# facebookresearch/mbrl-lib

Measured on AMD Instinct MI355X. Metric: candidate-steps/sec (pop×particles×horizon / plan) per CEM iter; plans/sec, higher is better.
Workload: dtype f32

## Files before the change

mbrl-lib_amd/csrc/cem.hpp:

```cpp
#pragma once
#include <type_traits>

#include "common.hpp"
#include "particle_reduce.hpp"

namespace hipets {

struct CemDev {
    int n_env;
    int pop, H, A, D;
    int K;
    float alpha, one_minus_alpha;
    int return_mean, clipped, unbiased;
    const float* totals = nullptr;
    int P = 0;
    ParticleReduce reduce{};
    const int* elite_in = nullptr;
};

__device__ __forceinline__ float philox_trunc_normal(uint32_t idx_lo, uint32_t idx_hi, uint64_t seed, uint64_t stream) {
    for (uint32_t attempt = 0; attempt < 64; ++attempt) {
        const Philox4 r = philox4x32_10(idx_lo, idx_hi, attempt, (uint32_t)stream, (uint32_t)seed,
                                        (uint32_t)(seed >> 32) ^ (uint32_t)(stream >> 32) ^ 0x5EED5EEDu);
        float n0, n1, n2, n3;
        box_muller(r.x, r.y, n0, n1);
        if (fabsf(n0) <= 2.0f) return n0;
        if (fabsf(n1) <= 2.0f) return n1;
        box_muller(r.z, r.w, n2, n3);
        if (fabsf(n2) <= 2.0f) return n2;
        if (fabsf(n3) <= 2.0f) return n3;
    }
    return 0.0f;
}

__device__ __forceinline__ float philox_normal(uint32_t idx_lo, uint32_t idx_hi, uint64_t seed, uint64_t stream) {
    const Philox4 r = philox4x32_10(idx_lo, idx_hi, 0u, (uint32_t)stream, (uint32_t)seed,
                                    (uint32_t)(seed >> 32) ^ (uint32_t)(stream >> 32) ^ 0x5EED5EEDu);
    float n0, n1;
    box_muller(r.x, r.y, n0, n1);
    return n0;
}

__global__ void cem_sample_kernel(const CemDev p, const float* __restrict__ mu, const float* __restrict__ disp,
                                  const float* __restrict__ lower, const float* __restrict__ upper,
                                  const float* __restrict__ z_in, unsigned long long seed, unsigned long long stream,
                                  float* __restrict__ population) {
    const long long i = (long long)blockIdx.x * blockDim.x + threadIdx.x;
    if (i >= (long long)p.n_env * p.pop * p.D) return;
    const int d = (int)(i % p.D);
    const int env = (int)(i / ((long long)p.pop * p.D));
    const float m = mu[env * p.D + d], v = disp[env * p.D + d], lb = lower[d], ub = upper[d];
    float x;
    if (p.clipped) {
        const float z = z_in ? z_in[i] : philox_normal((uint32_t)i, (uint32_t)(i >> 32), seed, stream);
        x = m + v * z;
        x = x > lb ? x : lb;
        x = x < ub ? x : ub;
    } else {
        const float lbd = (m - lb) / 2.0f, ubd = (ub - m) / 2.0f;
        const float mv = fminf(lbd * lbd, ubd * ubd);
        const float cv = fminf(mv, v);
        const float z = z_in ? z_in[i] : philox_trunc_normal((uint32_t)i, (uint32_t)(i >> 32), seed, stream);
        x = z * sqrtf(cv) + m;
    }
    population[i] = x;
}

#ifndef HIPETS_REFIT_SKIP
#define HIPETS_REFIT_SKIP 0
#endif
constexpr int kRefitThreads = 1024;
constexpr int kMaxPop = 8192;
constexpr int kRefitScratchBytes = 12288;
constexpr int kSelectMaxK = 1024;
constexpr int kRankSortMax = 640;

__global__ __launch_bounds__(kRefitThreads) void cem_refit_kernel(const CemDev p, float* values, const float* population, float* mu,
                                                                 float* disp, float* best_value, float* best_solution,
                                                                 int* elite_idx_out) {
    extern __shared__ __attribute__((aligned(16))) char smem[];
    {
        const int env = blockIdx.y;
        values += (size_t)env * p.pop;
        if (p.totals && !(HIPETS_REFIT_SKIP & 1)) {
            const float* tot = p.totals + (size_t)env * p.pop * p.P;
            for (int i = threadIdx.x; i < p.pop; i += kRefitThreads) values[i] = particle_value(tot + (size_t)i * p.P, 1, p.P, p.reduce);
        }
        population += (size_t)env * p.pop * p.D;
        mu += (size_t)env * p.D;
        disp += (size_t)env * p.D;
        best_value += env;
        best_solution += (size_t)env * p.D;
        if (elite_idx_out) elite_idx_out += (size_t)env * p.K;
    }
    const int* const elite_in = p.elite_in ? p.elite_in + (size_t)blockIdx.y * p.K : nullptr;
    int n2 = 1;
    while (n2 < p.pop) n2 <<= 1;
    float* key = reinterpret_cast<float*>(smem);
    int* idx = reinterpret_cast<int*>(smem + (size_t)n2 * 4);
    const int tid = threadIdx.x;
    for (int i = tid; i < n2; i += kRefitThreads) {
        float v = -INFINITY;
        if (i < p.pop) {
            v = values[i];
            if (v != v) { v = -1e-10f; values[i] = v; }
        }
        key[i] = v;
        idx[i] = i < p.pop ? i : 0x7FFFFFFF;
    }
    __syncthreads();
    if (elite_in) {
        auto in_range = [&](const int e) { return e < 0 ? 0 : (e >= p.pop ? p.pop - 1 : e); };
        const float top_key = key[in_range(elite_in[0])];
        __syncthreads();
        for (int k = tid; k < p.K; k += kRefitThreads) idx[k] = in_range(elite_in[k]);
        if (tid == 0) key[0] = top_key;
        __syncthreads();
    } else if (HIPETS_REFIT_SKIP & 2) {
    } else if (p.pop <= kRankSortMax) {
        for (int i = tid; i < p.pop; i += kRefitThreads) {
            const float ki = key[i];
            int rank = 0;
#pragma unroll 8
            for (int j = 0; j < i; ++j) rank += key[j] >= ki;
#pragma unroll 8
            for (int j = i + 1; j < p.pop; ++j) rank += key[j] > ki;
            idx[i] = rank;
        }
        __syncthreads();
        int* pos = reinterpret_cast<int*>(smem + (size_t)n2 * 8);
        for (int i = tid; i < p.pop; i += kRefitThreads) pos[idx[i]] = i;
        __syncthreads();
        float top_key = key[pos[0]];
        __syncthreads();
        for (int i = tid; i < p.pop; i += kRefitThreads) idx[i] = pos[i];
        if (tid == 0) key[0] = top_key;
        __syncthreads();
    } else if (p.K <= kSelectMaxK) {
        int* hist = reinterpret_cast<int*>(smem + (size_t)n2 * 8);
        int* ctl = hist + 256;
        int* elist = ctl + 8;
        float* ekey = reinterpret_cast<float*>(elist + kSelectMaxK);
        auto okey = [](float v) {
            const unsigned u = __float_as_uint(v + 0.0f);
            return (u & 0x80000000u) ? ~u : (u | 0x80000000u);
        };
        if (tid == 0) { ctl[0] = 0; ctl[1] = 0; ctl[2] = p.K; ctl[3] = 0; }
        for (int pass = 3; pass >= 0; --pass) {
            for (int b = tid; b < 256; b += kRefitThreads) hist[b] = 0;
            __syncthreads();
            const unsigned prefix = (unsigned)ctl[0], mask = (unsigned)ctl[1];
            for (int i = tid; i < p.pop; i += kRefitThreads) {
                const unsigned u = okey(key[i]);
                if ((u & mask) == prefix) atomicAdd(&hist[(u >> (8 * pass)) & 255u], 1);
            }
            __syncthreads();
            if (tid < 64) {
                const int h0 = hist[4 * tid], h1 = hist[4 * tid + 1], h2 = hist[4 * tid + 2], h3 = hist[4 * tid + 3];
                const int mine = h0 + h1 + h2 + h3;
                int above = mine;
#pragma unroll
                for (int d = 1; d < 64; d <<= 1) {
                    const int o = __shfl_down(above, d, 64);
                    if (tid + d < 64) above += o;
                }
                const int need = ctl[2];
                const int higher = above - mine;
                if (higher < need && need <= above) {
                    int n = need - higher, b = 4 * tid + 3;
// ... 40 lines not shown
        __syncthreads();
        if (my_pos >= 0) idx[my_pos] = my_id;
        if (my_pos == 0) key[0] = my_key;
        __syncthreads();
    } else
    for (int k = 2; k <= n2; k <<= 1) {
        for (int j = k >> 1; j > 0; j >>= 1) {
            for (int i = tid; i < n2; i += kRefitThreads) {
                const int ixj = i ^ j;
                if (ixj > i) {
                    const float ka = key[i], kb = key[ixj];
                    const int ia = idx[i], ib = idx[ixj];
                    const bool a_first = (ka > kb) || (ka == kb && ia < ib);
                    const bool up = (i & k) == 0;
                    if (up ? !a_first : a_first) {
                        key[i] = kb; key[ixj] = ka;
                        idx[i] = ib; idx[ixj] = ia;
                    }
                }
            }
            __syncthreads();
        }
    }
    if (elite_idx_out && blockIdx.x == 0)
        for (int k = tid; k < p.K; k += kRefitThreads) elite_idx_out[k] = idx[k];

    const float top = key[0];
    const bool improved = blockIdx.x == 0 && top > best_value[0];
    const int top_i = idx[0];
    __syncthreads();

    double* red = reinterpret_cast<double*>(smem + (size_t)n2 * 8);
    const int nb = (int)gridDim.x, bx = (int)blockIdx.x;
    const int Dslice = (((p.D + nb - 1) / nb + 63) / 64) * 64;
    const int d_lo = bx * Dslice, d_hi = min(p.D, d_lo + Dslice);
    int parts = kRefitThreads / Dslice;
    parts = parts < 1 ? 1 : (parts > 8 ? 8 : parts);
    const int G = kRefitThreads / parts;
    const int part = tid / G, dloc = tid % G;
    const int nu = (p.K + parts - 1) / parts;
    auto sweep = [&](const int base, auto nu_tag, auto hold_tag) __attribute__((always_inline)) {
        constexpr int NU = decltype(nu_tag)::value;
        constexpr bool HOLD = decltype(hold_tag)::value;
        const int d = base + dloc;
        const bool live = d < d_hi && part < parts;
        float mu_old = 0.f, disp_old = 0.f;
        float xv[NU];
        double s = 0.0;
        if (live) {
            if (part == 0) { mu_old = mu[d]; disp_old = disp[d]; }
            for (int k0 = part; k0 < (HOLD ? part + 1 : p.K); k0 += parts * NU) {
#pragma unroll
                for (int u = 0; u < NU; ++u) xv[u] = population[(size_t)idx[min(k0 + u * parts, p.K - 1)] * p.D + d];
#pragma unroll
                for (int u = 0; u < NU; ++u)
                    if (k0 + u * parts < p.K) s += (double)xv[u];
            }
        }
// ... 8 lines not shown
        double ss = 0.0;
        if (live) {
            for (int k0 = part; k0 < (HOLD ? part + 1 : p.K); k0 += parts * NU) {
                if constexpr (!HOLD) {
#pragma unroll
                    for (int u = 0; u < NU; ++u) xv[u] = population[(size_t)idx[min(k0 + u * parts, p.K - 1)] * p.D + d];
                }
#pragma unroll
                for (int u = 0; u < NU; ++u)
                    if (k0 + u * parts < p.K) {
                        const double dv = (double)xv[u] - mean;
                        ss += dv * dv;
                    }
            }
        }
        red[tid] = ss;
        __syncthreads();
        if (live && part == 0) {
            double var = 0.0;
            for (int q = 0; q < parts; ++q) var += red[q * G + dloc];
            var /= (double)(p.unbiased ? (p.K - 1) : p.K);
            const float new_mu = (float)mean;
            const float new_disp = p.clipped ? (float)sqrt(var) : (float)var;
            mu[d] = p.alpha * mu_old + p.one_minus_alpha * new_mu;
            disp[d] = p.alpha * disp_old + p.one_minus_alpha * new_disp;
        }
        __syncthreads();
    };
    constexpr int kBestHold = 4;
    float best_row[kBestHold];
    const bool best_held = p.D <= kBestHold * kRefitThreads;
    if (improved && best_held) {
#pragma unroll
        for (int u = 0; u < kBestHold; ++u) best_row[u] = population[(size_t)top_i * p.D + min(tid + u * kRefitThreads, p.D - 1)];
    }
    for (int base = d_lo; base < ((HIPETS_REFIT_SKIP & 4) ? d_lo : d_hi); base += G) {
        using T = std::true_type;
        using F = std::false_type;
        if (nu <= 2) sweep(base, std::integral_constant<int, 2>{}, T{});
        else if (nu <= 4) sweep(base, std::integral_constant<int, 4>{}, T{});
        else if (nu <= 8) sweep(base, std::integral_constant<int, 8>{}, T{});
        else if (nu <= 16) sweep(base, std::integral_constant<int, 16>{}, T{});
        else sweep(base, std::integral_constant<int, 16>{}, F{});
    }
    if (improved) {
        if (best_held) {
#pragma unroll
            for (int u = 0; u < kBestHold; ++u)
                if (tid + u * kRefitThreads < p.D) best_solution[tid + u * kRefitThreads] = best_row[u];
        } else {
            for (int d = tid; d < p.D; d += kRefitThreads) best_solution[d] = population[(size_t)top_i * p.D + d];
        }
        if (tid == 0) best_value[0] = top;
    }
}

inline int refit_blocks(const int D) { return D <= 128 ? 1 : (D + 127) / 128 > 8 ? 8 : (D + 127) / 128; }

__global__ void cem_init_kernel(const CemDev p, const float* x0, const float* lower, const float* upper, float* mu,
                                float* disp, float* best_value) {
    const int i = blockIdx.x * blockDim.x + threadIdx.x;
    if (i < p.n_env * p.D) {
        const int d = i % p.D;
        mu[i] = x0[i];
        const float w = upper[d] - lower[d];
        disp[i] = p.clipped ? 1.0f : (w * w) / 16.0f;
    }
    if (i < p.n_env) best_value[i] = -INFINITY;
}

}
```

mbrl-lib_amd/csrc/engine.hip:

```cpp
#include <cstdarg>
#include <cstdio>
#include <cstring>

#include "engine.hpp"

namespace hipets {

thread_local std::string g_err;
thread_local int g_err_kind = HIPETS_ERR_NONE;

int fail(const char* fmt, ...) {
    char buf[1024];
    va_list ap;
    va_start(ap, fmt);
    vsnprintf(buf, sizeof(buf), fmt, ap);
    va_end(ap);
    g_err = buf;
    g_err_kind = HIPETS_ERR_INVALID_ARGUMENT;
    return 1;
}

int fail_kind(const int kind, const char* fmt, ...) {
    char buf[1024];
    va_list ap;
// ... 69 lines not shown
    HCHECK(hipGetDeviceProperties(&prop, device));
    if (std::string(prop.gcnArchName).rfind("gfx950", 0) != 0)
        return fail("device %d is %s; libhipets is built for gfx950 (MI355X) only", device, prop.gcnArchName);
    auto* e = new hipets_engine();
    e->device = device;
    e->num_cu = prop.multiProcessorCount > 0 ? prop.multiProcessorCount : 256;
    e->lds_max = prop.sharedMemPerBlockOptin > 0 ? (size_t)prop.sharedMemPerBlockOptin : (size_t)prop.sharedMemPerBlock;
    if (e->lds_max > 160 * 1024) e->lds_max = 160 * 1024;
    if (hipHostMalloc(reinterpret_cast<void**>(&e->error_flag), sizeof(int), hipHostMallocMapped) != hipSuccess) e->error_flag = nullptr;
    if (e->error_flag) *e->error_flag = 0;
    const char* np = std::getenv("HIPETS_NO_PERSISTENT");
    e->persistent_ok = e->error_flag != nullptr && !(np && np[0] == '1');
    if (e->census.ensure(2 * sizeof(int))) e->persistent_ok = false;
    *out = e;
    return 0;
}

void hipets_destroy(hipets_engine* e) {
    if (!e) return;
    (void)hipSetDevice(e->device);
    comm_release(e);
    for (DevBuf* b : {&e->w3pack, &e->wpack, &e->bpack, &e->layer_meta, &e->norm_mean, &e->norm_std, &e->min_lv, &e->max_lv, &e->no_delta, &e->members,
                      &e->s0, &e->state, &e->totals, &e->term, &e->exchange, &e->step_keys, &e->plan_keys, &e->mu, &e->disp, &e->population, &e->values,
                      &e->best_value, &e->best_solution, &e->past_action, &e->kept, &e->elite_idx, &e->keep_idx, &e->planet_w, &e->planet_b, &e->planet_member, &e->planet_ops, &e->shard_values, &e->gathered, &e->census, &e->train_slab, &e->train_partial,
                      &e->policy.w, &e->policy.b, &e->compact_counts, &e->sac_ws, &e->sac_one, &e->critic.w, &e->critic.b,
                      &e->ensemble.w, &e->ensemble.b, &e->ensemble.norm, &e->ensemble.lv, &e->ensemble.cols})
        b->release();
    for (auto& ev : e->events) { (void)hipEventDestroy(ev.first); (void)hipEventDestroy(ev.second); }
    for (auto& ev : e->event_pool) { (void)hipEventDestroy(ev.first); (void)hipEventDestroy(ev.second); }
    if (e->error_flag) (void)hipHostFree(e->error_flag);
    if (e->last_done) (void)hipEventDestroy(e->last_done);
    for (auto& sl : e->stage) {
        if (sl.p) (void)hipHostFree(sl.p);
        if (sl.done) (void)hipEventDestroy(sl.done);
    }
    delete e;
}

int hipets_set_plan_mode(hipets_engine* e, int32_t mode) {
    if (!e) return fail("null engine");
    if (mode != HIPETS_MODE_FAST && mode != HIPETS_MODE_DEVICE) return fail("plan mode must be HIPETS_MODE_FAST or HIPETS_MODE_DEVICE");
    e->plan_mode = mode;
    return 0;
}

int hipets_set_particle_reduce(hipets_engine* e, int32_t kind, float kappa, int32_t worst_k) {
    if (!e) return fail("null engine");
// ... 74 lines not shown
```

mbrl-lib_amd/csrc/engine.hpp:

```cpp
#pragma once
#include <hip/hip_runtime.h>

#include <cstdlib>
#include <string>
#include <utility>
#include <vector>

#include "../../include/hipets.h"
#include "particle_reduce.hpp"
#include "planet_types.hpp"
#include "rollout_types.hpp"

namespace hipets {

extern thread_local std::string g_err;
extern thread_local int g_err_kind;

}

#pragma GCC visibility push(hidden)

namespace hipets {

int fail(const char* fmt, ...);
// ... 58 lines not shown
    int num_cu = 256;
    size_t lds_max = 160 * 1024;
    bool has_model = false;
    hipets::ModelDev md{};
    int ensemble_size = 0;
    DevBuf w3pack;
    DevBuf wpack, bpack, layer_meta, norm_mean, norm_std, min_lv, max_lv, no_delta, members;
    DevBuf s0, state, totals, term;
    DevBuf exchange, step_keys, plan_keys;
    struct HostStage { void* p = nullptr; size_t cap = 0; hipEvent_t done = nullptr; bool used = false; };
    HostStage stage[4];
    int stage_next = 0;
    uint32_t tag_base = 0;
    uint64_t plan_keys_seed = 0, plan_keys_first = 0;
    int plan_keys_count = 0, plan_keys_H = 0;
    int* error_flag = nullptr;
    bool persistent_ok = true;
    long long poll_ticks = 20000000ll;
    DevBuf census;
    hipStream_t last_stream = nullptr;
    bool last_stream_set = false;
    hipEvent_t last_done = nullptr;
    DevBuf mu, disp, population, values, best_value, best_solution, past_action, kept, elite_idx, keep_idx;
    void* comm = nullptr;
    int comm_rank = 0, comm_world = 1;
    DevBuf shard_values, gathered;
    bool has_planet = false;
    bool planet_static = false;
    hipets::PlanetDev pd{};
    DevBuf planet_w, planet_b, planet_member, planet_ops;
    int plan_mode = HIPETS_MODE_FAST;
    hipets::ParticleReduce reduce{};
    bool has_trace = false;
    hipets_plan_trace trace{};
    bool timing = false;
    int timing_stride = 1;
    unsigned long long launch_counter = 0;
    std::vector<std::pair<hipEvent_t, hipEvent_t>> events;
    std::vector<std::pair<hipEvent_t, hipEvent_t>> event_pool;
    DevBuf train_slab, train_partial;
    hipets::MlpSnapshot policy, critic;
    DevBuf compact_counts;
    bool has_sac = false;
    hipets::SacBind sac{};
    int sac_last_batch = 0;
    DevBuf sac_ws, sac_one;
// ... 22 lines not shown
    int kind = HIPETS_ERR_NONE;
    bool ok() const { return kind == HIPETS_ERR_NONE; }
    void note(const int rc) {
        if (rc && ok()) { msg = g_err; kind = g_err_kind == HIPETS_ERR_NONE ? HIPETS_ERR_RUNTIME : g_err_kind; }
    }
    int report() const {
        if (ok()) return 0;
        g_err = msg;
        g_err_kind = kind;
        return 1;
    }
};

int check_reduce(const hipets_engine* e, int P);


int launch_particle_reduce(const hipets_engine* e, const float* totals, float* returns, int pop, int P, hipStream_t st);

int rollout_impl(hipets_engine* e, const float* actions, const float* s0, int32_t pop, int32_t H, int32_t P, const hipets_rollout_opts* o,
                 float* returns, void* stream);
int planet_rollout_impl(hipets_engine* e, const float* actions, const float* latent0, const float* belief0, int32_t pop, int32_t H, int32_t P,
                        const hipets_planet_opts* o, float* returns, hipStream_t st);
int plan_step_keys(hipets_engine* e, int H, int iters, uint64_t seed, uint64_t first_stream, hipStream_t st);
int pack_weights(hipStream_t st, float* dst, const float* src, const int* members, int M, int K, int N, int Kp, int Np, long long member_stride,
                 long long layer_off, int permute_cols, int src_nk, int head_dim = 0);
int pack_weights_b3(hipStream_t st, uint4* dst, const float* src, const int* members, int M, int K, int N, int Kp32, int Np, long long member_stride,
                    long long layer_off, int src_nk, int pieces);
int pack_bias(hipStream_t st, float* dst, const float* src, const int* members, int M, int N, int Np, int member_stride, int layer_off,
              int permute_cols, int head_dim = 0);


int comm_all_gather(hipets_engine* e, size_t width, hipStream_t st);
int comm_unpad_shards(hipets_engine* e, int rows, int width, hipStream_t st);
void comm_release(hipets_engine* e);

}

#pragma GCC visibility pop
```

mbrl-lib_amd/csrc/plan.hip:

```cpp
#include <algorithm>
#include <cmath>
#include <vector>

#include "engine.hpp"
#include "lds_optin.hpp"
#include "optim.hpp"

using namespace hipets;

namespace {

int launch_mppi_sample(int n_env, int pop, int H, int A, float beta, const float* mean, const float* past_action, const float* lower, const float* upper,
                       const float* z, uint64_t seed, uint64_t stream_id, float* population, hipStream_t st) {
    const long long npop = (long long)n_env * pop;
    const long long D = (long long)H * A;
    if (D <= kMppiSampleMaxD) {
        const int G = mppi_sample_group(npop, (int)D);
        hipLaunchKernelGGL(mppi_sample_staged_kernel, dim3((unsigned)((npop + G - 1) / G)), dim3(kMppiSampleThreads), (size_t)G * D * 4, st, n_env, pop, H, A, G, beta,
                           mean, past_action, lower, upper, z, (unsigned long long)seed, (unsigned long long)stream_id, population);
    } else {
        const long long n = npop * A;
        hipLaunchKernelGGL(mppi_sample_kernel, dim3((unsigned)((n + 255) / 256)), dim3(256), 0, st, n_env, pop, H, A, beta, mean, past_action, lower, upper, z,
                           (unsigned long long)seed, (unsigned long long)stream_id, population);
    }
// ... 149 lines not shown
    return o;
}
PlanObjective planet_objective(const float* latent0, const float* belief0) {
    PlanObjective o;
    o.kind = PlanObjective::PLANET;
    o.latent0 = latent0;
    o.belief0 = belief0;
    return o;
}

int check_plan(const hipets_engine* e, const PlanObjective& obj, bool args, int A, int n_env, int P) {
    const bool planet = obj.is_planet();
    if (planet && !(e && e->has_planet)) return fail("engine has no PlaNet model (call hipets_planet_set_model)");
    if (!planet && !(e && e->has_model)) return fail("engine has no model (call hipets_set_model)");
    if (!args || (planet ? !(obj.latent0 && obj.belief0) : !obj.s0)) return fail("null argument");
    if (planet && A != e->pd.action) return fail("act_dim %d != model action_size %d", A, e->pd.action);
    if (!planet && A != e->md.act_dim) return fail("act_dim %d != model act_dim %d", A, e->md.act_dim);
    if (n_env < 1 || n_env > 4096) return fail("n_env %d outside [1, 4096]", n_env);
    if (planet && P < 1) return fail("bad pop/horizon/particles");
    return check_reduce(e, P);
}

int launch_cem_refit(const CemDev& c, float* values, const float* population, float* mu, float* disp, float* best_value, float* best_solution,
                     int* elite_idx, hipStream_t st) {
    int n2 = 1;
    while (n2 < c.pop) n2 <<= 1;
    hipLaunchKernelGGL(cem_refit_kernel, dim3(refit_blocks(c.D), c.n_env), dim3(kRefitThreads), (size_t)n2 * 8 + kRefitScratchBytes, st, c, values,
                       population, mu, disp, best_value, best_solution, elite_idx);
    HCHECK(hipGetLastError());
    return 0;
}

struct PlanLoop {
    int n_env, H, P, iters;
    uint64_t first_stream, stream_stride, rollout_stream;
    const float* population;
    float* returns;
};
template <class Prologue, class Rows, class Sample, class Refit>
int run_plan(hipets_engine* e, const PlanObjective& obj, const PlanLoop& pl, uint64_t seed, void* stream, Prologue prologue, Rows rows, Sample sample,
             Refit refit) {
    hipets_rollout_opts ro{};
    ro.mode = e->plan_mode;
    ro.seed = obj.rollout_seed(e, seed);
    ro.n_env = pl.n_env;
    const bool carry_on = obj.is_sharded();
    LocalErr le;
    le.note(prologue(ro.seed));
    for (int i = 0; i < pl.iters && (carry_on || le.ok()); ++i) {
        const uint64_t sid = (pl.first_stream + (uint64_t)i) * pl.stream_stride;
        if (le.ok()) le.note(sample(i, sid));
        ro.stream_id = sid + pl.rollout_stream;
        if (obj.evaluate(e, pl.population, rows(i), pl.H, pl.P, &ro, pl.returns, stream, le)) return 1;
        if (le.ok()) le.note(refit(i));
    }
    return le.report();
}

int plan_cem_impl(hipets_engine* e, const hipets_cem_params* p, int32_t n_env, const float* x0, const float* lower, const float* upper,
                  const PlanObjective& obj, int32_t P, uint64_t seed, uint64_t plan_id, float* out, void* stream) {
    if (check_cem(p) || check_plan(e, obj, x0 && lower && upper && out, p->act_dim, n_env, P)) return 1;
    if (obj.is_sharded() && check_shards(e, p->population_size, P)) return 1;
    hipStream_t st = reinterpret_cast<hipStream_t>(stream);
    HCHECK(hipSetDevice(e->device));
    ENTER_STREAM(e, st);
    const CemDev c = make_cem(p, n_env);
    const size_t nd = (size_t)n_env * c.D, npop = (size_t)n_env * c.pop;
    if (e->mu.ensure(nd * 4) || e->disp.ensure(nd * 4) || e->best_solution.ensure(nd * 4) || e->best_value.ensure((size_t)n_env * 4 + 16) ||
        e->population.ensure(npop * c.D * 4) || e->values.ensure(npop * 4) || obj.reserve_shards(e, c.pop))
        return 1;
    const int iters = p->num_iterations;
    const PlanLoop pl{n_env, c.H, P, iters, plan_id * (uint64_t)iters, 1, 0, e->population.as<float>(), nullptr};
    auto prologue = [&](uint64_t rollout_seed) -> int {
        if (obj.clear_padding(e, c.pop, st)) return 1;
        hipLaunchKernelGGL(cem_init_kernel, dim3((unsigned)((nd + 255) / 256)), dim3(256), 0, st, c, x0, lower, upper, e->mu.as<float>(),
                           e->disp.as<float>(), e->best_value.as<float>());
        HCHECK(hipGetLastError());
        HCHECK(hipMemsetAsync(e->best_solution.p, 0, nd * 4, st));
        return obj.is_planet() ? 0 : plan_prologue(e, obj.s0, n_env, c.H, iters, rollout_seed, pl.first_stream, st);
    };
    auto sample = [&](int, uint64_t sid) -> int {
        const long long n = (long long)npop * c.D;
        hipLaunchKernelGGL(cem_sample_kernel, dim3((unsigned)((n + 255) / 256)), dim3(256), 0, st, c, e->mu.as<float>(), e->disp.as<float>(),
                           lower, upper, (const float*)nullptr, (unsigned long long)seed, (unsigned long long)sid, e->population.as<float>());
        HCHECK(hipGetLastError());
        return 0;
    };
    auto refit = [&](int i) -> int {
        int* eidx = (e->has_trace && e->trace.elite_idx) ? e->trace.elite_idx + (size_t)i * n_env * c.K : nullptr;
        CemDev cr = c;
        obj.refit_from_totals(e, &cr, P);
        if (launch_cem_refit(cr, e->values.as<float>(), e->population.as<float>(), e->mu.as<float>(), e->disp.as<float>(), e->best_value.as<float>(),
                             e->best_solution.as<float>(), eidx, st))
            return 1;
        return trace_iter(e, i, (int)npop, (size_t)c.D, e->population.as<float>(), e->values.as<float>(), e->mu.as<float>(), e->disp.as<float>(), st, n_env);
    };
    if (run_plan(e, obj, pl, seed, stream, prologue, [&](int) { return (int)npop; }, sample, refit)) return 1;
    HCHECK(hipMemcpyAsync(out, p->return_mean_elites ? e->mu.p : e->best_solution.p, nd * 4, hipMemcpyDeviceToDevice, st));
    return 0;
}

int plan_mppi_impl(hipets_engine* e, int32_t pop, int32_t H, int32_t A, int32_t num_iterations, double gamma, double beta, int32_t n_env,
                   float* mean, const float* lower, const float* upper, const PlanObjective& obj, int32_t P, uint64_t seed, uint64_t plan_id,
                   void* stream) {
    if (check_plan(e, obj, mean && lower && upper, A, n_env, P)) return 1;
    if (pop < 1 || pop > 12000) return fail("population_size %d outside [1, 12000]", pop);
    if (H < 1 || num_iterations < 0) return fail("bad horizon/num_iterations");
    if (obj.is_sharded() && check_shards(e, pop, P)) return 1;
    hipStream_t st = reinterpret_cast<hipStream_t>(stream);
    HCHECK(hipSetDevice(e->device));
    ENTER_STREAM(e, st);
    const size_t nd = (size_t)H * A, npop = (size_t)n_env * pop;
    if (e->mu.ensure(n_env * nd * 4) || e->past_action.ensure((size_t)n_env * A * 4) || e->population.ensure(npop * nd * 4) ||
        e->values.ensure(npop * 4) || obj.reserve_shards(e, pop))
        return 1;
    const PlanLoop pl{n_env, H, P, num_iterations, plan_id * (uint64_t)num_iterations, 1, 0, e->population.as<float>(), e->values.as<float>()};
    auto prologue = [&](uint64_t rollout_seed) -> int {
        if (obj.clear_padding(e, pop, st)) return 1;
        HCHECK(hipMemcpyAsync(e->mu.p, mean, n_env * nd * 4, hipMemcpyDeviceToDevice, st));
        hipLaunchKernelGGL(mppi_shift_kernel, dim3((unsigned)((n_env * nd + 255) / 256)), dim3(256), 0, st, n_env, H, A, e->mu.as<float>(), mean,
                           e->past_action.as<float>());
// ... 297 lines not shown
```

mbrl-lib_amd/csrc/rollout.hip:

```cpp
#include <hip/hip_ext.h>

#include <algorithm>

#include "engine.hpp"
#include "launch.hpp"
#include "residency.hpp"
#include "returns_kernel.hpp"
#include "rollout_helpers.hpp"
#include "rollout_smem.hpp"

using namespace hipets;

namespace {

KernelRec* rollout_instance(const hipets_engine* e, int R, const RolloutArgs& ra) {
    static constexpr decltype(&rollout_instance_r1) resolvers[kMaxR] = {rollout_instance_r1, rollout_instance_r2, rollout_instance_r3, rollout_instance_r4};
    if (R < 1 || R > kMaxR) return fail("unsupported rows_per_group %d (1..%d)", R, kMaxR), nullptr;
    hipError_t why = hipSuccess;
    KernelRec* k = resolvers[R - 1](e->md, ra, &why);
    const bool b3 = e->md.precision == HIPETS_PREC_BF16X3;
    if (!k && why == hipErrorNotSupported && (b3 || e->md.precision == HIPETS_PREC_BF16))
        fail("precision %s: no shape-specialised kernel instance for this model / call (SiLU, f64 normaliser, no obs preprocessing, in-kernel "
             "sampling, one of the %s layer shapes, R = %d); use precision f32", b3 ? "bf16x3" : "bf16", b3 ? "BASELINE" : "two bf16", R);
    else if (!k) fail_kind(HIPETS_ERR_RUNTIME, "rollout kernel launch failed: %s", hipGetErrorString(why));
// ... 179 lines not shown
int pack_weights_b3(hipStream_t st, uint4* dst, const float* src, const int* members, int M, int K, int N, int Kp32, int Np, long long member_stride,
                    long long layer_off, int src_nk, int pieces) {
    const long long n3 = (long long)(Np / 16) * (Kp32 / 32) * pieces * 64 * M;
    hipLaunchKernelGGL(pack_weights_b3_kernel, dim3((unsigned)((n3 + 255) / 256)), dim3(256), 0, st, dst, src, members, M, K, N, Kp32, Np, member_stride,
                       layer_off, src_nk, pieces);
    HCHECK(hipGetLastError());
    return 0;
}

int pack_bias(hipStream_t st, float* dst, const float* src, const int* members, int M, int N, int Np, int member_stride, int layer_off, int permute_cols,
              int head_dim) {
    const int nb = M * Np;
    hipLaunchKernelGGL(pack_bias_kernel, dim3((nb + 255) / 256), dim3(256), 0, st, dst, src, members, M, N, Np, member_stride, layer_off, permute_cols, head_dim);
    HCHECK(hipGetLastError());
    return 0;
}

int launch_particle_reduce(const hipets_engine* e, const float* totals, float* returns, int pop, int P, hipStream_t st) {
    hipLaunchKernelGGL(particle_mean_kernel, dim3((pop + 255) / 256), dim3(256), 0, st, totals, returns, pop, P, e->reduce);
    HCHECK(hipGetLastError());
    return 0;
}

int plan_step_keys(hipets_engine* e, int H, int iters, uint64_t seed, uint64_t first_stream, hipStream_t st) {
    if (e->md.propagation != HIPETS_PROP_RANDOM_MODEL || iters < 1 || e->plan_mode != HIPETS_MODE_DEVICE || !e->persistent_ok) return 0;
    if (e->plan_keys.ensure((size_t)iters * H * sizeof(PermKeys))) return 1;
    hipLaunchKernelGGL(step_keys_kernel, dim3((H + 63) / 64, iters), dim3(64), 0, st, e->plan_keys.as<PermKeys>(), H, (unsigned long long)seed,
                       (unsigned long long)first_stream);
    HCHECK(hipGetLastError());
    e->plan_keys_seed = seed; e->plan_keys_first = first_stream; e->plan_keys_count = iters; e->plan_keys_H = H;
    return 0;
}

int rollout_impl(hipets_engine* e, const float* actions, const float* s0, int32_t pop, int32_t H, int32_t P,
                 const hipets_rollout_opts* o, float* returns, void* stream) {
    if (!e || !e->has_model) return fail("engine has no model (call hipets_set_model)");
    if (!actions || !o) return fail("null argument");
    if (pop < 1 || H < 1 || P < 1) return fail("bad pop/horizon/particles");
    if (check_reduce(e, P)) return 1;
    if (e->error_flag && *e->error_flag) {
        *e->error_flag = 0;
        e->persistent_ok = false;
        return fail_kind(HIPETS_ERR_TIMEOUT, "a persistent DEVICE-mode rollout timed out waiting for rows of another workgroup (its workgroups were not all "
                    "resident) and nobody asked (hipets_check_async_error after the results were read): the results of that earlier "
                    "call are invalid.  Persistent launches are now disabled for this engine.");
    }
    hipStream_t st = reinterpret_cast<hipStream_t>(stream);
    HCHECK(hipSetDevice(e->device));
    const ModelDev& md = e->md;
    const long long B = (long long)pop * P;
    if (B > 0x7FFFFFFF / std::max(md.obs_dim, md.out_dim)) return fail("batch too large");
    if (o->rows_per_group < 0 || o->rows_per_group > kMaxR) return fail("rows_per_group outside [0, %d]", kMaxR);

// ... 314 lines not shown
```

Baseline: 290.5 million.

## Fuse CEM sampling into refit and prologue with double-buffered populations

```diff
diff --git a/mbrl-lib_amd/csrc/cem.hpp b/mbrl-lib_amd/csrc/cem.hpp
--- a/mbrl-lib_amd/csrc/cem.hpp
+++ b/mbrl-lib_amd/csrc/cem.hpp
@@ -2,6 +2,7 @@
 #include <type_traits>
 
 #include "common.hpp"
+#include "draw_table.hpp"
 #include "particle_reduce.hpp"
 
 namespace hipets {
@@ -41,6 +42,22 @@
     return n0;
 }
 
+__device__ __forceinline__ float cem_draw(const int clipped, const long long i, const uint64_t seed, const uint64_t stream) {
+    return clipped ? philox_normal((uint32_t)i, (uint32_t)(i >> 32), seed, stream) : philox_trunc_normal((uint32_t)i, (uint32_t)(i >> 32), seed, stream);
+}
+
+__device__ __forceinline__ float cem_candidate(const int clipped, const float m, const float v, const float lb, const float ub, const float z) {
+    if (clipped) {
+        float x = m + v * z;
+        x = x > lb ? x : lb;
+        return x < ub ? x : ub;
+    }
+    const float lbd = (m - lb) / 2.0f, ubd = (ub - m) / 2.0f;
+    const float mv = fminf(lbd * lbd, ubd * ubd);
+    const float cv = fminf(mv, v);
+    return z * sqrtf(cv) + m;
+}
+
 __global__ void cem_sample_kernel(const CemDev p, const float* __restrict__ mu, const float* __restrict__ disp,
                                   const float* __restrict__ lower, const float* __restrict__ upper,
                                   const float* __restrict__ z_in, unsigned long long seed, unsigned long long stream,
@@ -50,21 +67,38 @@
     const int d = (int)(i % p.D);
     const int env = (int)(i / ((long long)p.pop * p.D));
     const float m = mu[env * p.D + d], v = disp[env * p.D + d], lb = lower[d], ub = upper[d];
-    float x;
-    if (p.clipped) {
-        const float z = z_in ? z_in[i] : philox_normal((uint32_t)i, (uint32_t)(i >> 32), seed, stream);
-        x = m + v * z;
-        x = x > lb ? x : lb;
-        x = x < ub ? x : ub;
-    } else {
-        const float lbd = (m - lb) / 2.0f, ubd = (ub - m) / 2.0f;
-        const float mv = fminf(lbd * lbd, ubd * ubd);
-        const float cv = fminf(mv, v);
-        const float z = z_in ? z_in[i] : philox_trunc_normal((uint32_t)i, (uint32_t)(i >> 32), seed, stream);
-        x = z * sqrtf(cv) + m;
-    }
-    population[i] = x;
-}
+    const float z = z_in ? z_in[i] : cem_draw(p.clipped, i, seed, stream);
+    population[i] = cem_candidate(p.clipped, m, v, lb, ub, z);
+}
+
+struct CemNext {
+    float* population = nullptr;
+    float* out = nullptr;
+    float* best_value = nullptr;
+    float* mu = nullptr;
+    float* disp = nullptr;
+    const float* lower = nullptr;
+    const float* upper = nullptr;
+    const float* z = nullptr;
+    unsigned long long seed = 0, stream = 0;
+};
+
+struct CemPrologue {
+    const float* x0 = nullptr;
+    const float* lower = nullptr;
+    const float* upper = nullptr;
+    float* mu = nullptr;
+    float* disp = nullptr;
+    float* best_value = nullptr;
+    float* best_solution = nullptr;
+    float* population = nullptr;
+    float* z = nullptr;
+    int iters = 0;
+    unsigned long long seed = 0, first_stream = 0;
+    PermKeys* keys = nullptr;
+    int key_iters = 0;
+    unsigned long long key_seed = 0, key_first_stream = 0;
+};
 
 #ifndef HIPETS_REFIT_SKIP
 #define HIPETS_REFIT_SKIP 0
@@ -75,38 +109,77 @@
 constexpr int kSelectMaxK = 1024;
 constexpr int kRankSortMax = 640;
 
+__device__ __forceinline__ unsigned order_key(const float v) {
+    const unsigned u = __float_as_uint(v + 0.0f);
+    return (u & 0x80000000u) ? ~u : (u | 0x80000000u);
+}
+
+constexpr int kRefitMeanQuads = 8;
+__device__ __forceinline__ float refit_value(const float* t, const int P, const ParticleReduce r) {
+    if (r.kind != HIPETS_REDUCE_MEAN || (P & 3) || P > 4 * kRefitMeanQuads) return particle_value(t, 1, P, r);
+    const float4* t4 = reinterpret_cast<const float4*>(t);
+    float4 q[kRefitMeanQuads];
+#pragma unroll
+    for (int u = 0; u < kRefitMeanQuads; ++u) q[u] = t4[min(u, P / 4 - 1)];
+    float s = 0.f;
+#pragma unroll
+    for (int u = 0; u < kRefitMeanQuads; ++u)
+        if (4 * u < P) {
+            s += q[u].x;
+            s += q[u].y;
+            s += q[u].z;
+            s += q[u].w;
+        }
+    return s / (float)P;
+}
+
+__host__ __device__ inline int refit_dslice(const int D, const int nb) { return (((D + nb - 1) / nb + 63) / 64) * 64; }
+
 __global__ __launch_bounds__(kRefitThreads) void cem_refit_kernel(const CemDev p, float* values, const float* population, float* mu,
                                                                  float* disp, float* best_value, float* best_solution,
-                                                                 int* elite_idx_out) {
+                                                                 int* elite_idx_out, CemNext nx) {
     extern __shared__ __attribute__((aligned(16))) char smem[];
+    const float* totals = nullptr;
+    const long long env_elem0 = (long long)blockIdx.y * p.pop * p.D;
     {
         const int env = blockIdx.y;
         values += (size_t)env * p.pop;
-        if (p.totals && !(HIPETS_REFIT_SKIP & 1)) {
-            const float* tot = p.totals + (size_t)env * p.pop * p.P;
-            for (int i = threadIdx.x; i < p.pop; i += kRefitThreads) values[i] = particle_value(tot + (size_t)i * p.P, 1, p.P, p.reduce);
-        }
+        if (p.totals && !(HIPETS_REFIT_SKIP & 1)) totals = p.totals + (size_t)env * p.pop * p.P;
         population += (size_t)env * p.pop * p.D;
         mu += (size_t)env * p.D;
         disp += (size_t)env * p.D;
         best_value += env;
         best_solution += (size_t)env * p.D;
         if (elite_idx_out) elite_idx_out += (size_t)env * p.K;
-    }
+        if (nx.population) nx.population += (size_t)env * p.pop * p.D;
+        if (nx.out) nx.out += (size_t)env * p.D;
+        if (nx.best_value) nx.best_value += env;
+        nx.mu = nx.mu ? nx.mu + (size_t)env * p.D : mu;
+        nx.disp = nx.disp ? nx.disp + (size_t)env * p.D : disp;
+    }
+    const bool writer = blockIdx.z == 0;
     const int* const elite_in = p.elite_in ? p.elite_in + (size_t)blockIdx.y * p.K : nullptr;
     int n2 = 1;
     while (n2 < p.pop) n2 <<= 1;
     float* key = reinterpret_cast<float*>(smem);
     int* idx = reinterpret_cast<int*>(smem + (size_t)n2 * 4);
     const int tid = threadIdx.x;
-    for (int i = tid; i < n2; i += kRefitThreads) {
+    const bool by_rank = !elite_in && !(HIPETS_REFIT_SKIP & 2) && p.pop <= kRankSortMax;
+    unsigned* ukey = reinterpret_cast<unsigned*>(smem + (((size_t)n2 * 8 + 15) & ~(size_t)15));
+    const int nq = (p.pop + 3) / 4;
+    for (int i = tid; i < (n2 > 4 * nq ? n2 : 4 * nq); i += kRefitThreads) {
         float v = -INFINITY;
         if (i < p.pop) {
-            v = values[i];
-            if (v != v) { v = -1e-10f; values[i] = v; }
-        }
-        key[i] = v;
-        idx[i] = i < p.pop ? i : 0x7FFFFFFF;
+            v = totals ? refit_value(totals + (size_t)i * p.P, p.P, p.reduce) : values[i];
+            const bool nan = v != v;
+            if (nan) v = -1e-10f;
+            if (blockIdx.x == 0 && writer && (totals || nan)) values[i] = v;
+        }
+        if (i < n2) {
+            key[i] = v;
+            idx[i] = i < p.pop ? i : 0x7FFFFFFF;
+        }
+        if (by_rank && i < 4 * nq) ukey[i] = i < p.pop ? order_key(v) : 0u;
     }
     __syncthreads();
     if (elite_in) {
@@ -117,34 +190,48 @@
         if (tid == 0) key[0] = top_key;
         __syncthreads();
     } else if (HIPETS_REFIT_SKIP & 2) {
-    } else if (p.pop <= kRankSortMax) {
-        for (int i = tid; i < p.pop; i += kRefitThreads) {
-            const float ki = key[i];
-            int rank = 0;
-#pragma unroll 8
-            for (int j = 0; j < i; ++j) rank += key[j] >= ki;
-#pragma unroll 8
-            for (int j = i + 1; j < p.pop; ++j) rank += key[j] > ki;
-            idx[i] = rank;
-        }
-        __syncthreads();
-        int* pos = reinterpret_cast<int*>(smem + (size_t)n2 * 8);
-        for (int i = tid; i < p.pop; i += kRefitThreads) pos[idx[i]] = i;
-        __syncthreads();
-        float top_key = key[pos[0]];
-        __syncthreads();
-        for (int i = tid; i < p.pop; i += kRefitThreads) idx[i] = pos[i];
-        if (tid == 0) key[0] = top_key;
+    } else if (by_rank) {
+        const int groups = (p.pop + 63) / 64;
+        const int splits = (kRefitThreads / 64) / groups;
+        const int wave = __builtin_amdgcn_readfirstlane(tid >> 6);
+        const int g = wave % groups, s = wave / groups;
+        const int i = 64 * g + (tid & 63);
+        const int qs = (nq + splits - 1) / splits;
+        int* part = reinterpret_cast<int*>(ukey + 4 * ((kRankSortMax + 3) / 4));
+        int rank = 0;
+        const bool counting = s < splits;
+        if (counting) {
+            const unsigned ui = ukey[i < p.pop ? i : 0];
+            const int q_lo = s * qs, q_hi = min(nq, q_lo + qs);
+            auto count = [&](const int qa, const int qb, auto threshold) __attribute__((always_inline)) {
+#pragma unroll 4
+                for (int q = qa; q < qb; ++q) {
+                    const uint4 x = *reinterpret_cast<const uint4*>(ukey + 4 * q);
+                    rank += x.x > threshold(4 * q);
+                    rank += x.y > threshold(4 * q + 1);
+                    rank += x.z > threshold(4 * q + 2);
+                    rank += x.w > threshold(4 * q + 3);
+                }
+            };
+            const int own_lo = 16 * g, own_hi = 16 * g + 16;
+            count(q_lo, min(q_hi, own_lo), [&](int) { return ui - 1u; });
+            count(max(q_lo, own_lo), min(q_hi, own_hi), [&](const int j) { return j < i ? ui - 1u : ui; });
+            count(max(q_lo, own_hi), q_hi, [&](int) { return ui; });
+            if (s > 0) part[(s - 1) * 64 * groups + i] = rank;
+        }
+        if (splits > 1) __syncthreads();
+        if (counting && s == 0 && i < p.pop) {
+            for (int o = 1; o < splits; ++o) rank += part[(o - 1) * 64 * groups + i];
+            idx[rank] = i;
+            if (rank == 0) key[0] = key[i];
+        }
         __syncthreads();
     } else if (p.K <= kSelectMaxK) {
         int* hist = reinterpret_cast<int*>(smem + (size_t)n2 * 8);
         int* ctl = hist + 256;
         int* elist = ctl + 8;
         float* ekey = reinterpret_cast<float*>(elist + kSelectMaxK);
-        auto okey = [](float v) {
-            const unsigned u = __float_as_uint(v + 0.0f);
-            return (u & 0x80000000u) ? ~u : (u | 0x80000000u);
-        };
+        auto okey = [](float v) { return order_key(v); };
         if (tid == 0) { ctl[0] = 0; ctl[1] = 0; ctl[2] = p.K; ctl[3] = 0; }
         for (int pass = 3; pass >= 0; --pass) {
             for (int b = tid; b < 256; b += kRefitThreads) hist[b] = 0;
@@ -231,18 +318,23 @@
             __syncthreads();
         }
     }
-    if (elite_idx_out && blockIdx.x == 0)
+    if (elite_idx_out && blockIdx.x == 0 && writer)
         for (int k = tid; k < p.K; k += kRefitThreads) elite_idx_out[k] = idx[k];
 
     const float top = key[0];
-    const bool improved = blockIdx.x == 0 && top > best_value[0];
+    const bool out_best = nx.out && !p.return_mean && writer;
+    const float best_prev = (blockIdx.x == 0 || out_best) ? best_value[0] : 0.f;
+    const bool improved_here = top > best_prev;
+    const bool improved = blockIdx.x == 0 && writer && improved_here;
     const int top_i = idx[0];
     __syncthreads();
 
     double* red = reinterpret_cast<double*>(smem + (size_t)n2 * 8);
     const int nb = (int)gridDim.x, bx = (int)blockIdx.x;
-    const int Dslice = (((p.D + nb - 1) / nb + 63) / 64) * 64;
+    const int Dslice = refit_dslice(p.D, nb);
     const int d_lo = bx * Dslice, d_hi = min(p.D, d_lo + Dslice);
+    float* const next_mu = nx.population ? reinterpret_cast<float*>(smem + (size_t)n2 * 8 + kRefitScratchBytes) : nullptr;
+    float* const next_disp = next_mu + Dslice;
     int parts = kRefitThreads / Dslice;
     parts = parts < 1 ? 1 : (parts > 8 ? 8 : parts);
     const int G = kRefitThreads / parts;
@@ -297,8 +389,14 @@
             var /= (double)(p.unbiased ? (p.K - 1) : p.K);
             const float new_mu = (float)mean;
             const float new_disp = p.clipped ? (float)sqrt(var) : (float)var;
-            mu[d] = p.alpha * mu_old + p.one_minus_alpha * new_mu;
-            disp[d] = p.alpha * disp_old + p.one_minus_alpha * new_disp;
+            const float mu_d = p.alpha * mu_old + p.one_minus_alpha * new_mu;
+            const float disp_d = p.alpha * disp_old + p.one_minus_alpha * new_disp;
+            if (writer) {
+                nx.mu[d] = mu_d;
+                nx.disp[d] = disp_d;
+                if (nx.out && p.return_mean) nx.out[d] = mu_d;
+            }
+            if (next_mu) { next_mu[d - d_lo] = mu_d; next_disp[d - d_lo] = disp_d; }
         }
         __syncthreads();
     };
@@ -326,11 +424,52 @@
         } else {
             for (int d = tid; d < p.D; d += kRefitThreads) best_solution[d] = population[(size_t)top_i * p.D + d];
         }
-        if (tid == 0) best_value[0] = top;
+        if (tid == 0 && !nx.best_value) best_value[0] = top;
+    }
+    if (nx.best_value && bx == 0 && writer && tid == 0) nx.best_value[0] = improved ? top : best_prev;
+
+    const int w = d_hi - d_lo;
+    if (out_best) {
+        for (int d = d_lo + tid; d < d_hi; d += kRefitThreads) nx.out[d] = improved_here ? population[(size_t)top_i * p.D + d] : best_solution[d];
+    }
+    if (nx.population && w > 0 && !(HIPETS_REFIT_SKIP & 8)) {
+        constexpr int kNextHold = 16;
+        const int ct = min(kRefitThreads, ((w + 63) / 64) * 64), rows_per_pass = kRefitThreads / ct;
+        const int r_local = tid / ct, c0 = tid % ct;
+        const int r0 = (int)blockIdx.z * rows_per_pass + r_local, r_step = (int)gridDim.z * rows_per_pass;
+        if (r_local < rows_per_pass)
+            for (int dl = c0; dl < w; dl += ct) {
+                const float m = next_mu[dl], v = next_disp[dl], lb = nx.lower[d_lo + dl], ub = nx.upper[d_lo + dl];
+                if (!nx.z) {
+                    for (int c = r0; c < p.pop; c += r_step) {
+                        const size_t e = (size_t)c * p.D + d_lo + dl;
+                        nx.population[e] = cem_candidate(p.clipped, m, v, lb, ub, cem_draw(p.clipped, env_elem0 + (long long)e, nx.seed, nx.stream));
+                    }
+                    continue;
+                }
+                for (int cb = r0; cb < p.pop; cb += kNextHold * r_step) {
+                    float z[kNextHold];
+#pragma unroll
+                    for (int u = 0; u < kNextHold; ++u) z[u] = nx.z[env_elem0 + (long long)min(cb + u * r_step, p.pop - 1) * p.D + d_lo + dl];
+#pragma unroll
+                    for (int u = 0; u < kNextHold; ++u) {
+                        const int c = cb + u * r_step;
+                        if (c < p.pop) nx.population[(size_t)c * p.D + d_lo + dl] = cem_candidate(p.clipped, m, v, lb, ub, z[u]);
+                    }
+                }
+            }
     }
 }
 
 inline int refit_blocks(const int D) { return D <= 128 ? 1 : (D + 127) / 128 > 8 ? 8 : (D + 127) / 128; }
+inline int refit_replicas(const int n_env, const int pop, const int D, const int num_cu) {
+    const int nb = refit_blocks(D);
+    const long long per_slice = (long long)pop * refit_dslice(D, nb);
+    long long r = (per_slice + 8 * kRefitThreads - 1) / (8 * kRefitThreads);
+    const long long room = num_cu / ((long long)nb * n_env);
+    r = r > room ? room : r;
+    return (int)(r < 1 ? 1 : (r > 16 ? 16 : r));
+}
 
 __global__ void cem_init_kernel(const CemDev p, const float* x0, const float* lower, const float* upper, float* mu,
                                 float* disp, float* best_value) {
@@ -344,4 +483,41 @@
     if (i < p.n_env) best_value[i] = -INFINITY;
 }
 
-}
+constexpr int kCemPrologueThreads = 256;
+__global__ __launch_bounds__(kCemPrologueThreads) void cem_prologue_kernel(const CemDev p, const CemPrologue q) {
+    const long long g = (long long)blockIdx.x * kCemPrologueThreads + threadIdx.x;
+    const long long n = draw_block_elems(p.n_env, p.pop, p.D);
+    auto disp0 = [&](const int d) {
+        const float w = q.upper[d] - q.lower[d];
+        return p.clipped ? 1.0f : (w * w) / 16.0f;
+    };
+    if (g < (long long)p.n_env * p.D) {
+        q.mu[g] = q.x0[g];
+        q.disp[g] = disp0((int)(g % p.D));
+        q.best_solution[g] = 0.f;
+    }
+    if (g < p.n_env) q.best_value[g] = -INFINITY;
+    if (g < (long long)q.key_iters * p.H) {
+        const int it = (int)(g / p.H), t = (int)(g % p.H);
+        q.keys[g] = perm_round_keys(perm_key(q.key_seed, q.key_first_stream + (unsigned long long)it, (unsigned)t));
+    }
+    if (g < (q.z ? (long long)q.iters * n : (q.iters > 0 ? n : 0))) {
+        const long long it = g / n, i = g % n;
+        const float z = cem_draw(p.clipped, i, q.seed, q.first_stream + (unsigned long long)it);
+        if (q.z) q.z[g] = z;
+        if (it == 0) {
+            const int d = (int)(i % p.D);
+            const int env = (int)(i / ((long long)p.pop * p.D));
+            q.population[i] = cem_candidate(p.clipped, q.x0[(size_t)env * p.D + d], disp0(d), q.lower[d], q.upper[d], z);
+        }
+    }
+}
+inline long long cem_prologue_threads(const CemDev& p, const CemPrologue& q) {
+    const long long n = draw_block_elems(p.n_env, p.pop, p.D);
+    long long t = q.z ? (long long)q.iters * n : (q.iters > 0 ? n : 0);
+    if (t < (long long)p.n_env * p.D) t = (long long)p.n_env * p.D;
+    if (t < (long long)q.key_iters * p.H) t = (long long)q.key_iters * p.H;
+    return t;
+}
+
+}
diff --git a/mbrl-lib_amd/csrc/draw_table.hpp b/mbrl-lib_amd/csrc/draw_table.hpp
--- /dev/null
+++ b/mbrl-lib_amd/csrc/draw_table.hpp
@@ -0,0 +1,29 @@
+#pragma once
+#include <cstddef>
+#include <cstdint>
+
+#if defined(__HIPCC__)
+#define HIPETS_HD __host__ __device__
+#else
+#define HIPETS_HD
+#endif
+
+namespace hipets {
+
+constexpr uint64_t kDrawTableCapBytes = 16ull << 20;
+
+HIPETS_HD inline int64_t draw_flat_index(int64_t env, int64_t candidate, int64_t d, int64_t pop, int64_t D) { return (env * pop + candidate) * D + d; }
+
+HIPETS_HD inline int64_t draw_block_elems(int64_t n_env, int64_t pop, int64_t D) { return n_env * pop * D; }
+
+HIPETS_HD inline int64_t draw_table_index(int64_t it, int64_t env, int64_t candidate, int64_t d, int64_t n_env, int64_t pop, int64_t D) {
+    return it * draw_block_elems(n_env, pop, D) + draw_flat_index(env, candidate, d, pop, D);
+}
+
+HIPETS_HD inline bool draw_table_fits(int64_t iters, int64_t block_elems, uint64_t cap_bytes) {
+    if (iters < 1 || block_elems < 1) return false;
+    const uint64_t cap_elems = cap_bytes / 4;
+    return (uint64_t)block_elems <= cap_elems / (uint64_t)iters;
+}
+
+}
diff --git a/mbrl-lib_amd/csrc/engine.hip b/mbrl-lib_amd/csrc/engine.hip
--- a/mbrl-lib_amd/csrc/engine.hip
+++ b/mbrl-lib_amd/csrc/engine.hip
@@ -115,7 +115,7 @@
     comm_release(e);
     for (DevBuf* b : {&e->w3pack, &e->wpack, &e->bpack, &e->layer_meta, &e->norm_mean, &e->norm_std, &e->min_lv, &e->max_lv, &e->no_delta, &e->members,
                       &e->s0, &e->state, &e->totals, &e->term, &e->exchange, &e->step_keys, &e->plan_keys, &e->mu, &e->disp, &e->population, &e->values,
-                      &e->best_value, &e->best_solution, &e->past_action, &e->kept, &e->elite_idx, &e->keep_idx, &e->planet_w, &e->planet_b, &e->planet_member, &e->planet_ops, &e->shard_values, &e->gathered, &e->census, &e->train_slab, &e->train_partial,
+                      &e->best_value, &e->best_solution, &e->past_action, &e->kept, &e->elite_idx, &e->keep_idx, &e->population_alt, &e->draws, &e->planet_w, &e->planet_b, &e->planet_member, &e->planet_ops, &e->shard_values, &e->gathered, &e->census, &e->train_slab, &e->train_partial,
                       &e->policy.w, &e->policy.b, &e->compact_counts, &e->sac_ws, &e->sac_one, &e->critic.w, &e->critic.b,
                       &e->ensemble.w, &e->ensemble.b, &e->ensemble.norm, &e->ensemble.lv, &e->ensemble.cols})
         b->release();
diff --git a/mbrl-lib_amd/csrc/engine.hpp b/mbrl-lib_amd/csrc/engine.hpp
--- a/mbrl-lib_amd/csrc/engine.hpp
+++ b/mbrl-lib_amd/csrc/engine.hpp
@@ -104,6 +104,7 @@
     bool last_stream_set = false;
     hipEvent_t last_done = nullptr;
     DevBuf mu, disp, population, values, best_value, best_solution, past_action, kept, elite_idx, keep_idx;
+    DevBuf population_alt, draws;
     void* comm = nullptr;
     int comm_rank = 0, comm_world = 1;
     DevBuf shard_values, gathered;
@@ -172,6 +173,7 @@
 int planet_rollout_impl(hipets_engine* e, const float* actions, const float* latent0, const float* belief0, int32_t pop, int32_t H, int32_t P,
                         const hipets_planet_opts* o, float* returns, hipStream_t st);
 int plan_step_keys(hipets_engine* e, int H, int iters, uint64_t seed, uint64_t first_stream, hipStream_t st);
+int plan_step_keys_reserve(hipets_engine* e, int H, int iters, uint64_t seed, uint64_t first_stream, PermKeys** keys);
 int pack_weights(hipStream_t st, float* dst, const float* src, const int* members, int M, int K, int N, int Kp, int Np, long long member_stride,
                  long long layer_off, int permute_cols, int src_nk, int head_dim = 0);
 int pack_weights_b3(hipStream_t st, uint4* dst, const float* src, const int* members, int M, int K, int N, int Kp32, int Np, long long member_stride,
diff --git a/mbrl-lib_amd/csrc/plan.hip b/mbrl-lib_amd/csrc/plan.hip
--- a/mbrl-lib_amd/csrc/plan.hip
+++ b/mbrl-lib_amd/csrc/plan.hip
@@ -195,13 +195,20 @@
 }
 
 int launch_cem_refit(const CemDev& c, float* values, const float* population, float* mu, float* disp, float* best_value, float* best_solution,
-                     int* elite_idx, hipStream_t st) {
+                     int* elite_idx, hipStream_t st, const CemNext& nx = CemNext{}, int replicas = 1) {
     int n2 = 1;
     while (n2 < c.pop) n2 <<= 1;
-    hipLaunchKernelGGL(cem_refit_kernel, dim3(refit_blocks(c.D), c.n_env), dim3(kRefitThreads), (size_t)n2 * 8 + kRefitScratchBytes, st, c, values,
-                       population, mu, disp, best_value, best_solution, elite_idx);
+    const int nb = refit_blocks(c.D);
+    const size_t smem = (size_t)n2 * 8 + kRefitScratchBytes + (nx.population ? (size_t)refit_dslice(c.D, nb) * 8 : 0);
+    hipLaunchKernelGGL(cem_refit_kernel, dim3(nb, c.n_env, replicas), dim3(kRefitThreads), smem, st, c, values, population, mu, disp, best_value, best_solution,
+                       elite_idx, nx);
     HCHECK(hipGetLastError());
     return 0;
+}
+
+uint64_t draw_table_cap() {
+    const char* s = std::getenv("HIPETS_DRAW_TABLE_CAP");
+    return s && *s ? std::strtoull(s, nullptr, 10) : kDrawTableCapBytes;
 }
 
 struct PlanLoop {
@@ -209,6 +216,7 @@
     uint64_t first_stream, stream_stride, rollout_stream;
     const float* population;
     float* returns;
+    const float* population_alt = nullptr;
 };
 template <class Prologue, class Rows, class Sample, class Refit>
 int run_plan(hipets_engine* e, const PlanObjective& obj, const PlanLoop& pl, uint64_t seed, void* stream, Prologue prologue, Rows rows, Sample sample,
@@ -224,7 +232,8 @@
         const uint64_t sid = (pl.first_stream + (uint64_t)i) * pl.stream_stride;
         if (le.ok()) le.note(sample(i, sid));
         ro.stream_id = sid + pl.rollout_stream;
-        if (obj.evaluate(e, pl.population, rows(i), pl.H, pl.P, &ro, pl.returns, stream, le)) return 1;
+        const float* population = (pl.population_alt && (i & 1)) ? pl.population_alt : pl.population;
+        if (obj.evaluate(e, population, rows(i), pl.H, pl.P, &ro, pl.returns, stream, le)) return 1;
         if (le.ok()) le.note(refit(i));
     }
     return le.report();
@@ -239,37 +248,66 @@
     ENTER_STREAM(e, st);
     const CemDev c = make_cem(p, n_env);
     const size_t nd = (size_t)n_env * c.D, npop = (size_t)n_env * c.pop;
-    if (e->mu.ensure(nd * 4) || e->disp.ensure(nd * 4) || e->best_solution.ensure(nd * 4) || e->best_value.ensure((size_t)n_env * 4 + 16) ||
-        e->population.ensure(npop * c.D * 4) || e->values.ensure(npop * 4) || obj.reserve_shards(e, c.pop))
+    const int iters = p->num_iterations;
+    const long long block = draw_block_elems(n_env, c.pop, c.D);
+    const bool table = draw_table_fits(iters, block, draw_table_cap());
+    if (e->mu.ensure(nd * 8) || e->disp.ensure(nd * 8) || e->best_solution.ensure(nd * 4) || e->best_value.ensure((size_t)n_env * 8 + 16) ||
+        e->population.ensure(npop * c.D * 4) || e->population_alt.ensure(npop * c.D * 4) || e->values.ensure(npop * 4) ||
+        (table && e->draws.ensure((size_t)iters * block * 4)) || obj.reserve_shards(e, c.pop))
         return 1;
-    const int iters = p->num_iterations;
-    const PlanLoop pl{n_env, c.H, P, iters, plan_id * (uint64_t)iters, 1, 0, e->population.as<float>(), nullptr};
+    float* const pop_of[2] = {e->population.as<float>(), e->population_alt.as<float>()};
+    float* const best_of[2] = {e->best_value.as<float>(), e->best_value.as<float>() + n_env};
+    float* const mu_of[2] = {e->mu.as<float>(), e->mu.as<float>() + nd};
+    float* const disp_of[2] = {e->disp.as<float>(), e->disp.as<float>() + nd};
+    const PlanLoop pl{n_env, c.H, P, iters, plan_id * (uint64_t)iters, 1, 0, pop_of[0], nullptr, pop_of[1]};
     auto prologue = [&](uint64_t rollout_seed) -> int {
         if (obj.clear_padding(e, c.pop, st)) return 1;
-        hipLaunchKernelGGL(cem_init_kernel, dim3((unsigned)((nd + 255) / 256)), dim3(256), 0, st, c, x0, lower, upper, e->mu.as<float>(),
-                           e->disp.as<float>(), e->best_value.as<float>());
-        HCHECK(hipGetLastError());
-        HCHECK(hipMemsetAsync(e->best_solution.p, 0, nd * 4, st));
-        return obj.is_planet() ? 0 : plan_prologue(e, obj.s0, n_env, c.H, iters, rollout_seed, pl.first_stream, st);
-    };
-    auto sample = [&](int, uint64_t sid) -> int {
-        const long long n = (long long)npop * c.D;
-        hipLaunchKernelGGL(cem_sample_kernel, dim3((unsigned)((n + 255) / 256)), dim3(256), 0, st, c, e->mu.as<float>(), e->disp.as<float>(),
-                           lower, upper, (const float*)nullptr, (unsigned long long)seed, (unsigned long long)sid, e->population.as<float>());
-        HCHECK(hipGetLastError());
+        CemPrologue q;
+        q.x0 = x0; q.lower = lower; q.upper = upper;
+        q.mu = mu_of[0]; q.disp = disp_of[0]; q.best_value = best_of[0]; q.best_solution = e->best_solution.as<float>();
+        q.population = pop_of[0];
+        q.z = table ? e->draws.as<float>() : nullptr;
+        q.iters = iters;
+        q.seed = seed; q.first_stream = pl.first_stream;
+        if (!obj.is_planet()) {
+            if (e->s0.ensure((size_t)n_env * e->md.obs_dim * 4) || stage_h2d(e, e->s0.p, obj.s0, (size_t)n_env * e->md.obs_dim * 4, st)) return 1;
+            if (plan_step_keys_reserve(e, c.H, iters, rollout_seed, pl.first_stream, &q.keys)) return 1;
+            if (q.keys) { q.key_iters = iters; q.key_seed = rollout_seed; q.key_first_stream = pl.first_stream; }
+        }
+        const long long threads = cem_prologue_threads(c, q);
+        hipLaunchKernelGGL(cem_prologue_kernel, dim3((unsigned)((threads + kCemPrologueThreads - 1) / kCemPrologueThreads)), dim3(kCemPrologueThreads), 0, st, c, q);
+        const hipError_t err = hipGetLastError();
+        if (err != hipSuccess) e->plan_keys_count = 0;
+        HCHECK(err);
         return 0;
     };
+    auto sample = [](int, uint64_t) -> int { return 0; };
     auto refit = [&](int i) -> int {
         int* eidx = (e->has_trace && e->trace.elite_idx) ? e->trace.elite_idx + (size_t)i * n_env * c.K : nullptr;
         CemDev cr = c;
         obj.refit_from_totals(e, &cr, P);
-        if (launch_cem_refit(cr, e->values.as<float>(), e->population.as<float>(), e->mu.as<float>(), e->disp.as<float>(), e->best_value.as<float>(),
-                             e->best_solution.as<float>(), eidx, st))
+        CemNext nx;
+        nx.best_value = best_of[(i + 1) & 1];
+        nx.mu = mu_of[(i + 1) & 1];
+        nx.disp = disp_of[(i + 1) & 1];
+        int replicas = 1;
+        if (i + 1 < iters) {
+            nx.population = pop_of[(i + 1) & 1];
+            nx.lower = lower; nx.upper = upper;
+            nx.z = table ? e->draws.as<float>() + (size_t)(i + 1) * block : nullptr;
+            nx.seed = seed; nx.stream = pl.first_stream + (uint64_t)(i + 1);
+            replicas = refit_replicas(n_env, c.pop, c.D, e->num_cu);
+        } else {
+            nx.out = out;
+        }
+        if (launch_cem_refit(cr, e->values.as<float>(), pop_of[i & 1], mu_of[i & 1], disp_of[i & 1], best_of[i & 1], e->best_solution.as<float>(), eidx, st,
+                             nx, replicas))
             return 1;
-        return trace_iter(e, i, (int)npop, (size_t)c.D, e->population.as<float>(), e->values.as<float>(), e->mu.as<float>(), e->disp.as<float>(), st, n_env);
+        return trace_iter(e, i, (int)npop, (size_t)c.D, pop_of[i & 1], e->values.as<float>(), nx.mu, nx.disp, st, n_env);
     };
     if (run_plan(e, obj, pl, seed, stream, prologue, [&](int) { return (int)npop; }, sample, refit)) return 1;
-    HCHECK(hipMemcpyAsync(out, p->return_mean_elites ? e->mu.p : e->best_solution.p, nd * 4, hipMemcpyDeviceToDevice, st));
+    if (iters < 1)
+        HCHECK(hipMemcpyAsync(out, p->return_mean_elites ? (void*)mu_of[0] : e->best_solution.p, nd * 4, hipMemcpyDeviceToDevice, st));
     return 0;
 }
 
diff --git a/mbrl-lib_amd/csrc/rollout.hip b/mbrl-lib_amd/csrc/rollout.hip
--- a/mbrl-lib_amd/csrc/rollout.hip
+++ b/mbrl-lib_amd/csrc/rollout.hip
@@ -225,13 +225,24 @@
     return 0;
 }
 
-int plan_step_keys(hipets_engine* e, int H, int iters, uint64_t seed, uint64_t first_stream, hipStream_t st) {
+int plan_step_keys_reserve(hipets_engine* e, int H, int iters, uint64_t seed, uint64_t first_stream, PermKeys** keys) {
+    *keys = nullptr;
     if (e->md.propagation != HIPETS_PROP_RANDOM_MODEL || iters < 1 || e->plan_mode != HIPETS_MODE_DEVICE || !e->persistent_ok) return 0;
     if (e->plan_keys.ensure((size_t)iters * H * sizeof(PermKeys))) return 1;
-    hipLaunchKernelGGL(step_keys_kernel, dim3((H + 63) / 64, iters), dim3(64), 0, st, e->plan_keys.as<PermKeys>(), H, (unsigned long long)seed,
+    e->plan_keys_seed = seed; e->plan_keys_first = first_stream; e->plan_keys_count = iters; e->plan_keys_H = H;
+    *keys = e->plan_keys.as<PermKeys>();
+    return 0;
+}
+
+int plan_step_keys(hipets_engine* e, int H, int iters, uint64_t seed, uint64_t first_stream, hipStream_t st) {
+    PermKeys* keys;
+    if (plan_step_keys_reserve(e, H, iters, seed, first_stream, &keys)) return 1;
+    if (!keys) return 0;
+    hipLaunchKernelGGL(step_keys_kernel, dim3((H + 63) / 64, iters), dim3(64), 0, st, keys, H, (unsigned long long)seed,
                        (unsigned long long)first_stream);
-    HCHECK(hipGetLastError());
-    e->plan_keys_seed = seed; e->plan_keys_first = first_stream; e->plan_keys_count = iters; e->plan_keys_H = H;
+    const hipError_t err = hipGetLastError();
+    if (err != hipSuccess) e->plan_keys_count = 0;
+    HCHECK(err);
     return 0;
 }
 
```

Result: no change. 291.6 million (median of 6 runs) (+0.4%).
